# meiqua/pose_refine

Hardware: AMD Instinct MI355X
Metric: refined poses/sec (640x480, 20 ICP iters) (higher is better)
Workload: dtype f32; 1 GPU; obj_06.ply, 256-pose batch per GPU, 640x480 synthetic depth, projective association, 20 ICP iterations (21 passes), solve on device, 2 pose groups; poses_per_gpu=256, global_batch=256, parallelism=pose-shard x1, no data-path collective, no gather (1 rank)

## Files before the change

### pose_refine_amd/csrc/icp_accumulate.h

```cpp
#pragma once
#include "nn_query.h"

namespace prk {

struct Acc29 { float2v pk[16]; };
__device__ constexpr int kAccLo[16] = { 0, 6, 2, 7, 3, 8, 5, 11, 12, 24, 14, 15, 18, 17, 20, 27 };
__device__ constexpr int kAccHi[16] = { 1, -1, 21, 22, 4, 9, 10, 23, 13, 25, 26, 16, -1, 19, -1, 28 };
__device__ __forceinline__ void acc_clear(Acc29 &a) {
#pragma unroll
    for (int i = 0; i < 16; ++i) a.pk[i] = float2v{ 0.0f, 0.0f };
}
__device__ __forceinline__ void acc_export(const Acc29 &a, float (&out)[29]) {
#pragma unroll
    for (int i = 0; i < 16; ++i) { if (kAccLo[i] >= 0) out[kAccLo[i]] = a.pk[i].x; if (kAccHi[i] >= 0) out[kAccHi[i]] = a.pk[i].y; }
}
#define PR_SEL(v, i, j) __builtin_shufflevector(v, v, i, j)
__device__ __forceinline__ void accumulate(Acc29 &acc, float sx, float sy, float sz, const Corr &c)
{
    const float ex = c.dx - sx, ey = c.dy - sy, ez = c.dz - sz;
    const float r = ex * c.nx + ey * c.ny + ez * c.nz;
    const float2v C01{ c.nz * sy - c.ny * sz, c.nx * sz - c.nz * sx };
    const float2v C2R{ c.ny * sx - c.nx * sy, r };
    const float2v N01{ c.nx, c.ny };
    const float2v N2Z{ c.nz, c.dz };
// ... 49 lines not shown
    acc.pk[9]  += PR_SEL(WC2R, 1, 1) * N01;
    acc.pk[10] += WC2R * PR_SEL(N2Z, 0, 0);
    acc.pk[11] += PR_SEL(WN01, 0, 0) * N01;
    acc.pk[12] += PR_SEL(WN01, 1, 1) * PR_SEL(N01, 1, 0);
    acc.pk[13] += WN01 * PR_SEL(N2Z, 0, 0);
    acc.pk[14] += PR_SEL(WN2Z, 0, 0) * N2Z;
    acc.pk[15] += float2v{ e2, 1.0f };
    return w;
}
__device__ __forceinline__ void robust_store_corr(float *row, bool valid, const Corr &c, float w)
{
    const float4 a = valid ? make_float4(c.dx, c.dy, c.dz, 1.0f) : make_float4(0.0f, 0.0f, 0.0f, 0.0f);
    const float4 b = valid ? make_float4(c.nx, c.ny, c.nz, w) : make_float4(0.0f, 0.0f, 0.0f, 0.0f);
    reinterpret_cast<float4 *>(row)[0] = a;
    reinterpret_cast<float4 *>(row)[1] = b;
}
#undef PR_SEL

__device__ __forceinline__ void accumulate_score(Acc29 &acc, float sx, float sy, float sz, const Corr &c)
{
    const float ex = c.dx - sx, ey = c.dy - sy, ez = c.dz - sz;
    const float e2 = ex * ex + ey * ey + ez * ez;
    acc.pk[15] += float2v{ e2, 1.0f };
}


template <bool kScoreOnly, bool kRobust>
__device__ __forceinline__ void accumulate_point(Acc29 &acc, float sx, float sy, float sz, const Corr &c, const RobustW &rb)
{
    if constexpr (kScoreOnly) accumulate_score(acc, sx, sy, sz, c);
    else if constexpr (kRobust) (void)accumulate_weighted(acc, sx, sy, sz, c, rb);
    else accumulate(acc, sx, sy, sz, c);
}
template <class Scene, bool kNN, int kStack, bool kScoreOnly = false, bool kRobust = false>
__device__ __forceinline__ void vb_accumulate_at(uint32_t tib, float (&acc_out)[29], float *cl, uint32_t n, uint32_t first, uint32_t steps, bool xf,
                                                 const float (&M)[12], const Scene &scene, const int4 *lds_topo, int *stk_node, float *stk_lb,
                                                 uint32_t *nn_prev = nullptr, bool nn_seeded = false, const RobustW &rb = RobustW{})
{
    (void)nn_prev; (void)nn_seeded; (void)rb;
    struct { uint32_t steps; } b{ steps };
    Acc29 acc;
    acc_clear(acc);
    uint32_t lane_winner = kNoPrev;
    (void)lane_winner;
    (void)lds_topo; (void)stk_node; (void)stk_lb;
    auto point_of = [&](uint32_t j0, uint32_t i) { return j0 + i * kBlockThreads; };
    auto load_step = [&](uint32_t s, float (&p)[12], uint32_t &j0, uint32_t &cnt) {
        j0 = first + s * kPointsPerStep + tib;
        cnt = (j0 >= n) ? 0u : (((n - j0 + kBlockThreads - 1u) / kBlockThreads < kPointsPerLane) ? (n - j0 + kBlockThreads - 1u) / kBlockThreads : kPointsPerLane);
        const uint32_t last = n - 1u;
#pragma unroll
        for (uint32_t i = 0; i < 4; ++i) {
            const uint32_t j = point_of(j0, i);
            const pr_vec3 v = ld_off<pr_vec3>(cl, (j < last ? j : last) * 12u);
            p[3 * i] = v.x; p[3 * i + 1] = v.y; p[3 * i + 2] = v.z;
        }
    };
    auto process_step = [&](float (&p)[12], uint32_t j0, uint32_t cnt) {
        if (cnt == 0) return;
        if ((!kNN || kStack != -1) && xf) {
            const float2v Mx{ M[0], M[4] }, My{ M[1], M[5] }, Mz{ M[2], M[6] }, Mt{ M[3], M[7] };
#pragma unroll
            for (int i = 0; i < 4; ++i) {
                const float x = p[3 * i], y = p[3 * i + 1], z = p[3 * i + 2];
                float2v t = Mx * float2v{ x, x };
                t = t + My * float2v{ y, y };
                t = t + Mz * float2v{ z, z };
                t = t + Mt;
                p[3 * i]     = t.x;
                p[3 * i + 1] = t.y;
                p[3 * i + 2] = M[8] * x + M[9] * y + M[10] * z + M[11];
            }
#if !PR_PASS_LATE_STORE
#pragma unroll
            for (uint32_t i = 0; i < 4; ++i)
                if (i < cnt) st_off<pr_vec3>(cl, point_of(j0, i) * 12u, pr_vec3{ p[3 * i], p[3 * i + 1], p[3 * i + 2] });
#endif
        }
        auto store_back = [&]() {
#if PR_PASS_LATE_STORE
            if ((!kNN || kStack != -1) && xf) {
#pragma unroll
                for (uint32_t i = 0; i < 4; ++i)
                    if (i < cnt) st_off<pr_vec3>(cl, point_of(j0, i) * 12u, pr_vec3{ p[3 * i], p[3 * i + 1], p[3 * i + 2] });
            }
#endif
        };
        if constexpr (kNN) store_back();
        if constexpr (kNN && kStack == -1) {
            uint32_t w[4];
#pragma unroll
            for (uint32_t i = 0; i < 4; ++i) w[i] = (i < cnt) ? scene.winner[point_of(j0, i)] : kNoPrev;
            float4 d[4]; float nx[4], ny[4], nz[4];
#pragma unroll
            for (uint32_t i = 0; i < 4; ++i) {
                const uint32_t at = (w[i] != kNoPrev) ? w[i] : 0u;
                d[i] = scene.pts[at];
                const float *n = reinterpret_cast<const float *>(scene.normal + at);
                nx[i] = n[0]; ny[i] = n[1]; nz[i] = n[2];
            }
#pragma unroll
            for (uint32_t i = 0; i < 4; ++i) {
                if (w[i] != kNoPrev) {
                    Corr c; c.dx = d[i].x; c.dy = d[i].y; c.dz = d[i].z; c.nx = nx[i]; c.ny = ny[i]; c.nz = nz[i];
                    accumulate_point<kScoreOnly, kRobust>(acc, p[3 * i], p[3 * i + 1], p[3 * i + 2], c, rb);
                }
            }
        } else if constexpr (kNN) {
#pragma unroll
            for (uint32_t i = 0; i < 4; ++i) {
                if (i < cnt) {
                    Corr c;
                    bool ok;
                    if constexpr (kStack > 0) {
                        const uint32_t seed = (nn_prev && nn_seeded) ? nn_prev[point_of(j0, i)] : kNoPrev;
                        uint32_t winner;
                        ok = query_nn_stack<kStack>(scene, reinterpret_cast<const float4 *>(lds_topo), stk_node, stk_lb, p[3 * i], p[3 * i + 1], p[3 * i + 2], c,
// ... 28 lines not shown
    };

#if PR_PASS_PREFETCH
    {
        float p[12];
        uint32_t j0, cnt;
        load_step(0, p, j0, cnt);
        for (uint32_t s = 0; s < b.steps && cnt != 0; ++s) {
            float pn[12];
            uint32_t j0n = 0, cntn = 0;
            if (s + 1 < b.steps) load_step(s + 1, pn, j0n, cntn);
            process_step(p, j0, cnt);
#pragma unroll
            for (int i = 0; i < 12; ++i) p[i] = pn[i];
            j0 = j0n; cnt = cntn;
        }
    }
#else
    for (uint32_t s = 0; s < b.steps; ++s) {
        float p[12];
        uint32_t j0, cnt;
        load_step(s, p, j0, cnt);
        if (cnt == 0) break;
        process_step(p, j0, cnt);
    }
#endif
    acc_export(acc, acc_out);
}
template <class Scene, bool kNN, int kStack, bool kScoreOnly = false, bool kRobust = false>
__device__ __forceinline__ void vb_accumulate(float (&acc_out)[29], float *cl, uint32_t n, uint32_t first, uint32_t steps, bool xf,
                                              const float (&M)[12], const Scene &scene, const int4 *lds_topo, int *stk_node, float *stk_lb,
                                              uint32_t *nn_prev = nullptr, bool nn_seeded = false, const RobustW &rb = RobustW{})
{
    vb_accumulate_at<Scene, kNN, kStack, kScoreOnly, kRobust>(threadIdx.x, acc_out, cl, n, first, steps, xf, M, scene, lds_topo, stk_node, stk_lb, nn_prev, nn_seeded, rb);
}

template <bool kScoreOnly = false>
__device__ __forceinline__ void wave_reduce(float (&acc)[29], uint32_t lane, float *row)
{
    constexpr int kFirst = kScoreOnly ? 27 : 0;
#if PR_PASS_TAIL_PRIO
    __builtin_amdgcn_s_setprio(PR_PASS_TAIL_PRIO);
#endif
    if constexpr (!kScoreOnly) {
        const bool b1 = (lane & 1u) != 0, b2 = (lane & 2u) != 0;
        float p1[16], p2[8], p3[4], p4[2];
#pragma unroll
        for (int i = 0; i < 29; ++i) acc[i] += dpp_get<0x111, 0xf>(acc[i]);
#pragma unroll
        for (int k = 0; k < 15; ++k) {
            const float hi = acc[2 * k], lo = (2 * k + 1 < 29) ? dpp_get<0x101, 0xf>(acc[2 * k + 1 < 29 ? 2 * k + 1 : 28]) : 0.0f;
            p1[k] = b1 ? hi : lo;
        }
        p1[15] = 0.0f;
#pragma unroll
        for (int k = 0; k < 15; ++k) p1[k] += dpp_get<0x112, 0xf>(p1[k]);
#pragma unroll
        for (int m = 0; m < 8; ++m) {
            const float lo = dpp_get<0x102, 0xf>(p1[2 * m + 1]);
            p2[m] = b2 ? p1[2 * m] : lo;
        }
#pragma unroll
        for (int m = 0; m < 8; ++m) p2[m] += dpp_get<0x114, 0xf>(p2[m]);
#pragma unroll
        for (int q = 0; q < 4; ++q)
            p3[q] = __int_as_float(__builtin_amdgcn_update_dpp(__float_as_int(p2[2 * q]), __float_as_int(p2[2 * q + 1]), 0x104, 0xf, 0x5, false));
#pragma unroll
// ... 42 lines not shown
```

### pose_refine_amd/csrc/icp_pass.hip

```cpp
#include "pr_launch.h"
#include "icp_accumulate.h"
#include "icp_solve_device.h"

namespace prk {

template <class Scene, bool kNN, int kStack = 0, bool kRobust = false>
__global__ __launch_bounds__(256, PR_PASS_WAVES) void icp_pass_kernel(IcpBatch b, Scene scene)
{
    extern __shared__ __attribute__((aligned(16))) unsigned char lds_raw[];
    __shared__ float wsum[4][kAccStride];

    const uint32_t pose = blockIdx.y;
    const PoseMeta &pm = b.meta[pose];
    const int32_t st = pm.state;
    if (st == kSkip) return;
    const uint32_t n = pm.count;
    const uint32_t ppb = b.steps * kPointsPerStep;
    if ((uint64_t)blockIdx.x * ppb >= n) return;

    const int4 *lds_topo = nullptr;
    int *stk_node = nullptr; float *stk_lb = nullptr;
    if constexpr (kNN && kStack == 0) {
        int4 *dst = reinterpret_cast<int4 *>(lds_raw);
        for (uint32_t i = threadIdx.x; i < scene.lds_nodes; i += kBlockThreads) dst[i] = scene.topo[i];
// ... 25 lines not shown
        for (int i = 0; i < 29; ++i) acc[i] = 0.0f;
        float t;
        if (b.score_only) {
            vb_accumulate<Scene, kNN, kStack, true>(acc, cl, n, vb * ppb, b.steps, xf, M, scene, lds_topo, stk_node, stk_lb, nn_prev, xf);
            t = vb_reduce<true>(acc, wsum);
        } else {
            if constexpr (kRobust)
                vb_accumulate<Scene, kNN, kStack, false, true>(acc, cl, n, vb * ppb, b.steps, xf, M, scene, lds_topo, stk_node, stk_lb, nn_prev, xf, RobustW{ b.robust_kind, b.robust_c, b.robust_inv_c });
            else
                vb_accumulate<Scene, kNN, kStack>(acc, cl, n, vb * ppb, b.steps, xf, M, scene, lds_topo, stk_node, stk_lb, nn_prev, xf);
            t = vb_reduce(acc, wsum);
        }
        if (pass_deliver(b, pose, vb, used, n, t)) return;
    }
}

__device__ __forceinline__ float sum_partials(const float *partial, uint32_t pose, uint32_t nblk, uint32_t used, uint32_t comp)
{
    float total = 0.0f;
    const float *p = partial + (size_t)pose * nblk * kAccStride + comp;
    for (uint32_t g0 = 0; g0 < used; g0 += 16) {
        float v[16];
#pragma unroll
        for (uint32_t k = 0; k < 16; ++k) v[k] = (g0 + k < used) ? p[(size_t)(g0 + k) * kAccStride] : 0.0f;
#pragma unroll
        for (uint32_t k = 0; k < 16; ++k) if (g0 + k < used) total += v[k];
    }
    return total;
}

constexpr uint32_t kLoopLanes = 1024, kLoopWaves = kLoopLanes / 64, kLoopHeader = 64;
static_assert(sizeof(DevIcpState) == 20 * sizeof(uint32_t), "the LDS header holds DevIcpState as 20 words");
size_t icp_loop_cu_lds_bytes(uint32_t nblk) { return ((size_t)nblk * 4 * kAccStride + kLoopHeader) * sizeof(float); }

template <class Scene>
__global__ __launch_bounds__(kLoopLanes) PR_LOOP_CU_ATTR void icp_loop_cu_kernel(IcpBatch b, Scene scene)
{
    extern __shared__ __attribute__((aligned(16))) float loop_lds[];
    const uint32_t pose = blockIdx.x;
    const PoseMeta &pm = b.meta[pose];
    const int32_t st0 = pm.state;
    const uint32_t n = pm.count;
    if (st0 == kSkip || n == 0) return;
    const uint32_t ppb = b.steps * kPointsPerStep;
    const uint32_t items = ((n + ppb - 1) / ppb) * 4u;
    const uint32_t lane = threadIdx.x & 63u;
    const uint32_t wave = __builtin_amdgcn_readfirstlane(threadIdx.x >> 6);
    float *hdr = loop_lds + (size_t)b.nblk * 4 * kAccStride;
    uint32_t *hdw = reinterpret_cast<uint32_t *>(hdr);
    float *cl = reinterpret_cast<float *>(b.cloud + pm.start);
    bool xf = (st0 == kRunWithTransform) && !b.pre_transformed;
    float M[12];
#pragma unroll
    for (int i = 0; i < 12; ++i) M[i] = xf ? pm.xform[i] : 0.0f;
    if (wave == 0 && lane < 20) hdw[16 + lane] = reinterpret_cast<const uint32_t *>(b.st + pose)[lane];

    const uint32_t last_it = (uint32_t)b.crit.max_iteration;
    uint32_t it = 0;
    for (;; ++it) {
        const bool score_only = it == last_it;
        for (uint32_t item = wave; item < items; item += kLoopWaves) {
            const uint32_t vb = item >> 2, tib = ((item & 3u) << 6) | lane;
            float acc[29];
            float *row = loop_lds + (size_t)item * kAccStride;
            if (score_only) {
                vb_accumulate_at<Scene, false, 0, true>(tib, acc, cl, n, vb * ppb, b.steps, xf, M, scene, nullptr, nullptr, nullptr, nullptr, xf);
                wave_reduce<true>(acc, lane, row);
            } else {
                vb_accumulate_at<Scene, false, 0>(tib, acc, cl, n, vb * ppb, b.steps, xf, M, scene, nullptr, nullptr, nullptr, nullptr, xf);
                wave_reduce(acc, lane, row);
            }
        }
        __syncthreads();
        if (wave == 0) {
            float total = 0.0f;
            if (lane < 29) {
                const float *r = loop_lds + lane;
                for (uint32_t i = 0; i < items; i += 4u, r += 4 * kAccStride)
                    total += ((r[0] + r[kAccStride]) + r[2 * kAccStride]) + r[3 * kAccStride];
            }
            DevIcpState s;
#pragma unroll
            for (int i = 0; i < 16; ++i) s.T[i] = hdr[16 + i];
            s.fitness = hdr[32]; s.rmse = hdr[33]; s.done = (int32_t)hdw[34]; s.passes = (int32_t)hdw[35];
            float E[16];
            const bool finished = pose_iteration_wave(total, n, s, b.crit, it, E);
            if (lane == 0) {
#pragma unroll
                for (int i = 0; i < 16; ++i) hdr[16 + i] = s.T[i];
                hdr[32] = s.fitness; hdr[33] = s.rmse; hdw[35] = (uint32_t)s.passes;
                if (!finished) {
#pragma unroll
                    for (int i = 0; i < 12; ++i) hdr[i] = E[i];
                }
                hdw[12] = (finished || it >= last_it) ? 1u : 0u;
            }
        }
        __syncthreads();
        if (__builtin_amdgcn_readfirstlane(hdw[12]) != 0u) break;
#pragma unroll
        for (int i = 0; i < 12; ++i) M[i] = __int_as_float(__builtin_amdgcn_readfirstlane(__float_as_int(hdr[i])));
        xf = true;
    }
    if (threadIdx.x == 0) {
        DevIcpState s;
#pragma unroll
        for (int i = 0; i < 16; ++i) s.T[i] = hdr[16 + i];
        s.fitness = hdr[32]; s.rmse = hdr[33]; s.done = 1; s.passes = (int32_t)hdw[35];
        b.st[pose] = s;
        PoseMeta *wm = const_cast<PoseMeta *>(b.meta) + pose;
        if (it > 0) {
#pragma unroll
            for (int i = 0; i < 12; ++i) wm->xform[i] = hdr[i];
        }
        wm->state = kSkip;
    }
}
hipError_t launch_icp_loop_cu_proj_packed(const IcpBatch &b, const SceneProjPacked &sc, uint32_t n_poses, hipStream_t s)
{
    if (n_poses == 0 || b.nblk == 0) return hipSuccess;
    const size_t lds = icp_loop_cu_lds_bytes(b.nblk);
    if (lds > kLoopCuLdsBudget || b.robust_kind != PR_ROBUST_NONE) return hipErrorInvalidValue;
    hipLaunchKernelGGL(HIP_KERNEL_NAME(icp_loop_cu_kernel<SceneProjPacked>), dim3(n_poses), dim3(kLoopLanes), lds, s, b, sc);
    return hipGetLastError();
}

__global__ __launch_bounds__(64) void icp_finalize_kernel(const float *__restrict__ partial, const PoseMeta *__restrict__ meta,
                                                          uint32_t nblk, uint32_t ppb, float *__restrict__ sums)
{
    const uint32_t pose = blockIdx.x;
    if (meta[pose].state == kSkip) return;
    const uint32_t n = meta[pose].count;
    const uint32_t used = (n + ppb - 1) / ppb;
    if (threadIdx.x < kAccStride)
        sums[(size_t)pose * kAccStride + threadIdx.x] = (threadIdx.x < 29) ? sum_partials(partial, pose, nblk, used, threadIdx.x) : 0.0f;
}

__global__ __launch_bounds__(64) void icp_finalize_solve_kernel(const float *__restrict__ partial, PoseMeta *__restrict__ meta,
                                                                uint32_t nblk, uint32_t ppb, DevIcpState *__restrict__ st,
                                                                pr_criteria crit, uint32_t iter)
{
    const uint32_t pose = blockIdx.x;
    if (meta[pose].state == kSkip) return;
    const uint32_t n = meta[pose].count;
    const uint32_t used = (n + ppb - 1) / ppb;
    DevIcpState s = st[pose];
    float total = 0.0f;
    if (threadIdx.x < 29) total = sum_partials(partial, pose, nblk, used, threadIdx.x);
    float E[16];
    const bool finished = pose_iteration_wave(total, n, s, crit, iter, E);
    if (threadIdx.x != 0) return;
    if (finished) { s.done = 1; meta[pose].state = kSkip; }
    else {
#pragma unroll
        for (int i = 0; i < 12; ++i) meta[pose].xform[i] = E[i];
        meta[pose].state = kRunWithTransform;
// ... 129 lines not shown
```

### pose_refine_amd/csrc/pr_context.cpp

```cpp
#include "pr_runtime.h"

namespace prh {
thread_local std::string g_err;
void set_error(const char *fmt, ...)
{
    char buf[512];
    va_list ap; va_start(ap, fmt); vsnprintf(buf, sizeof buf, fmt, ap); va_end(ap);
    g_err = buf;
}
}

namespace prr {

static std::mutex &g_reg_mu_trace() { static std::mutex m; return m; }

namespace {
struct TraceRec { uint64_t ns; const char *tag; uint32_t tid; };
constexpr size_t kTraceCap = 1u << 18;
TraceRec *g_trace = nullptr;
std::atomic<uint64_t> g_trace_n{ 0 };
std::atomic<int> g_trace_state{ 0 };
std::string g_trace_path;
void trace_dump()
{
    FILE *f = std::fopen(g_trace_path.c_str(), "w");
    if (!f) return;
    const uint64_t n = std::min<uint64_t>(g_trace_n.load(), kTraceCap);
    for (uint64_t i = 0; i < n; ++i) std::fprintf(f, "%llu %u %s\n", (unsigned long long)g_trace[i].ns, g_trace[i].tid, g_trace[i].tag);
    std::fclose(f);
}
}
void trace_mark(const char *tag)
{
    int st = g_trace_state.load(std::memory_order_acquire);
    if (st == 1) return;
    if (st == 0) {
        std::lock_guard<std::mutex> lk(g_reg_mu_trace());
        st = g_trace_state.load();
        if (st == 0) {
            const char *p = std::getenv("PR_TRACE");
            if (p && *p) { g_trace_path = p; g_trace = new TraceRec[kTraceCap]; std::atexit(trace_dump); st = 2; } else st = 1;
            g_trace_state.store(st, std::memory_order_release);
        }
        if (st == 1) return;
    }
    timespec ts; clock_gettime(CLOCK_MONOTONIC, &ts);
    static thread_local uint32_t tid = (uint32_t)std::hash<std::thread::id>()(std::this_thread::get_id());
    const uint64_t i = g_trace_n.fetch_add(1);
    if (i < kTraceCap) g_trace[i] = TraceRec{ (uint64_t)ts.tv_sec * 1000000000ull + (uint64_t)ts.tv_nsec, tag, tid };
}

WriteLog g_writes;
std::atomic<uint64_t> g_flag_overtook{ 0 };
std::atomic<uint64_t> g_tight_batches{ 0 };
std::atomic<uint64_t> g_band_batches{ 0 };
std::atomic<uint64_t> g_resident_batches{ 0 };
Options opt;
std::mutex g_reg_mu;
std::vector<Ctx *> g_shared;
int g_default_device = -1;
thread_local Ctx *g = nullptr;
thread_local PrivateCtx tl_private;
std::mutex g_private_mu;
std::vector<Ctx *> g_private;

void ctx_teardown(Ctx *c)
{
    if (!c->ready) return;
    (void)hipSetDevice(c->device);
    hipStreamSynchronize(c->stream);
    for (Slot &sl : c->slots) slot_release(sl);
    for (DevBuf *b : { &c->aabb, &c->aabb_keys, &c->bbox, &c->poses, &c->depth, &c->row_count, &c->row_off, &c->counts, &c->cloud, &c->meta, &c->partial,
                       &c->sums, &c->packed.rec, &c->nn_prev, &c->dstate, &c->dresults, &c->arrive, &c->conv16, &c->conv8, &c->kd_scratch, &c->kd_tmp, &c->nn_full, &c->gather_tmp, &c->nn_counters, &c->scores, &c->multi, &c->ov_bits, &c->ov_box, &c->ov_mat, &c->cov_state, &c->cov_claimed, &c->mesh_sorted, &c->mesh_verts, &c->contours, &c->normals, &c->cmp_keys, &c->cmp_box, &c->cmp_rec, &c->edge_bits, &c->edge_rows, &c->lvl_rows, &c->lvl_counts, &c->lvl_carry, &c->pd_mats, &c->pd_part, &c->pd_rec, &c->ppf_tmp, &c->ppf_out, &c->plane_tmp, &c->seg_tmp, &c->dfilt_tmp, &c->vsd_rec, &c->solid_far, &c->solid_rec, &c->info_meta, &c->info_part }) b->release();
    for (NNDerived &d : c->nn_sets) d.release();
    for (PinBuf *b : { &c->h_sums, &c->h_meta, &c->h_counts, &c->h_results, &c->h_dstate, &c->h_poses, &c->h_flags, &c->h_scores, &c->h_multi, &c->h_ov, &c->h_cov, &c->h_contours, &c->h_normals, &c->h_lvl_carry, &c->h_cmp, &c->h_pd_mats, &c->h_pd_rec, &c->h_ppf, &c->h_plane, &c->h_seg, &c->h_dfilt, &c->h_vsd, &c->h_solid, &c->h_info_meta, &c->h_info_out }) b->release();
    c->packed = PackedCache();
    for (auto &gr : c->graphs) destroy_graph(gr);
    c->graphs.clear();
    c->spans.destroy();
    for (auto &e : c->gather_ev) { hipEventDestroy(e.first); hipEventDestroy(e.second); }
    c->gather_ev.clear(); c->gather_ev_used = 0;
    hipStreamDestroy(c->stream);
    if (c->ev_fork) hipEventDestroy(c->ev_fork);
    c->ev_fork = nullptr;
    for (int i = 0; i < 3; ++i) {
        if (c->side[i]) hipStreamDestroy(c->side[i]);
        if (c->ev_join[i]) hipEventDestroy(c->ev_join[i]);
        c->side[i] = nullptr; c->ev_join[i] = nullptr;
    }
// ... 166 lines not shown
    note_write(dev_dst, count * sizeof(int32_t));
    HIP_TRY(prk::launch_fill_i32(dev_dst, count, value, g->stream));
    HIP_TRY(hipStreamSynchronize(g->stream));
    return PR_OK;
}

int pr_set_option(const char *name, int value)
{
    std::lock_guard<std::mutex> lk(g_reg_mu);
    if (!name) { set_error("pr_set_option: null name"); return PR_ERR_INVALID; }
    const std::string n(name);
    if (n == "solve") { if (value != PR_SOLVE_HOST && value != PR_SOLVE_DEVICE) { set_error("solve must be 0 or 1"); return PR_ERR_INVALID; } opt.solve_mode = value; }
    else if (n == "host_worker") opt.host_worker = value ? 1 : 0;
    else if (n == "start_overlap") opt.start_overlap = value;
    else if (n == "points_per_block") { if (value < 1024 || value % 1024) { set_error("points_per_block must be a multiple of 1024"); return PR_ERR_INVALID; } opt.steps = value / 1024; }
    else if (n == "profile") { if (value < 0 || value > 3) { set_error("profile must be 0, 1 (every launch, synchronous calls), 2 (every launch of one call in sample_period) or 3 (every launch, asynchronous batches stay asynchronous)"); return PR_ERR_INVALID; } opt.profile = value; }
    else if (n == "sample_period") opt.sample_period = std::max(1, value);
    else if (n == "scene_cache") opt.scene_cache = value ? 1 : 0;
    else if (n == "nn_lds_nodes") opt.nn_lds_nodes = std::max(0, value);
    else if (n == "nn_lds_records") opt.nn_lds_records = std::max(0, value);
    else if (n == "nn_compact") opt.nn_compact = value ? 1 : 0;
    else if (n == "nn_wide") opt.nn_wide = value ? 1 : 0;
    else if (n == "blocking_wait") opt.blocking_wait = value ? 1 : 0;
    else if (n == "nn_seed") opt.nn_seed = value ? 1 : 0;
    else if (n == "nn_stack") opt.nn_stack = value ? 1 : 0;
    else if (n == "nn_split") opt.nn_split = value ? 1 : 0;
    else if (n == "nn_run") opt.nn_run = std::min(256, std::max(1, value));
    else if (n == "nn_grid") opt.nn_grid = value ? 1 : 0;
    else if (n == "nn_count") opt.nn_count = value ? 1 : 0;
    else if (n == "host_poll") opt.host_poll = value ? 1 : 0;
    else if (n == "graph") opt.use_graph = value ? 1 : 0;
    else if (n == "fused_solve") opt.fused_solve = value ? 1 : 0;
    else if (n == "resident_loop") opt.resident_loop = value ? 1 : 0;
    else if (n == "sub_batch") opt.sub_batch = std::min(32768, std::max(32, value));
    else if (n == "overlap_pass") opt.overlap_pass = std::max(-1, value);
    else if (n == "pose_groups") opt.pose_groups = std::min(4, std::max(0, value));
    else if (n == "eager_streams") opt.eager_streams = value ? 1 : 0;
    else if (n == "mesh_order") opt.mesh_order = value ? 1 : 0;
    else if (n == "tight_box") opt.tight_box = value ? 1 : 0;
    else if (n == "box_bands") opt.box_bands = value ? 1 : 0;
    else if (n == "ppf_walk") opt.ppf_walk = value ? 1 : 0;
    else if (n == "raster_mode") { if (value < 0 || value > 1) { set_error("raster_mode must be 0 or 1"); return PR_ERR_INVALID; } opt.raster_mode = value; }
    else { set_error("unknown option %s", name); return PR_ERR_INVALID; }
    return PR_OK;
}

int pr_get_option(const char *name, int *value)
{
    std::lock_guard<std::mutex> lk(g_reg_mu);
    if (!name || !value) { set_error("pr_get_option: null argument"); return PR_ERR_INVALID; }
    const std::string n(name);
    if (n == "solve") *value = opt.solve_mode;
    else if (n == "host_worker") *value = opt.host_worker;
    else if (n == "start_overlap") *value = opt.start_overlap;
    else if (n == "points_per_block") *value = opt.steps * 1024;
    else if (n == "profile") *value = opt.profile;
    else if (n == "sample_period") *value = opt.sample_period;
    else if (n == "scene_cache") *value = opt.scene_cache;
    else if (n == "nn_lds_nodes") *value = opt.nn_lds_nodes;
    else if (n == "nn_lds_records") *value = opt.nn_lds_records;
    else if (n == "nn_compact") *value = opt.nn_compact;
    else if (n == "nn_wide") *value = opt.nn_wide;
    else if (n == "blocking_wait") *value = opt.blocking_wait;
    else if (n == "nn_seed") *value = opt.nn_seed;
    else if (n == "nn_stack") *value = opt.nn_stack;
    else if (n == "nn_split") *value = opt.nn_split;
    else if (n == "nn_run") *value = opt.nn_run;
    else if (n == "nn_grid") *value = opt.nn_grid;
    else if (n == "nn_count") *value = opt.nn_count;
    else if (n == "host_poll") *value = opt.host_poll;
    else if (n == "stat_flag_overtook") *value = (int)std::min<uint64_t>(g_flag_overtook.load(), 0x7fffffffull);
    else if (n == "stat_tight_batches") *value = (int)std::min<uint64_t>(g_tight_batches.load(), 0x7fffffffull);
    else if (n == "box_pack") *value = (int)prk::kBoxPack;
    else if (n == "pose_dist_chunk") *value = (int)prk::kPoseDistChunk;
    else if (n == "raster_mode") *value = opt.raster_mode;
    else if (n == "mesh_order") *value = opt.mesh_order;
    else if (n == "tight_box") *value = opt.tight_box;
    else if (n == "box_bands") *value = opt.box_bands;
    else if (n == "ppf_walk") *value = opt.ppf_walk;
    else if (n == "stat_band_batches") *value = (int)std::min<uint64_t>(g_band_batches.load(), 0x7fffffffull);
    else if (n == "eager_streams") *value = opt.eager_streams;
    else if (n == "graph") *value = opt.use_graph;
    else if (n == "fused_solve") *value = opt.fused_solve;
    else if (n == "resident_loop") *value = opt.resident_loop;
    else if (n == "stat_resident_batches") *value = (int)std::min<uint64_t>(g_resident_batches.load(), 0x7fffffffull);
    else if (n == "sub_batch") *value = opt.sub_batch;
    else if (n == "overlap_pass") *value = opt.overlap_pass;
    else if (n == "pose_groups") *value = opt.pose_groups;
    else { set_error("unknown option %s", name); return PR_ERR_INVALID; }
    return PR_OK;
}

int pr_profile_reset(void)
{
    PR_TRY(bind_default());
    std::lock_guard<std::mutex> lk(g->mu);
    g->icp_ms = g->render_ms = g->cloud_ms = 0; g->icp_launches = g->icp_points = g->icp_bytes = 0; g->sample_clock = 0;
    g->gather_ms = 0; g->gather_n = 0; g->gather_ev_used = 0;
    g->icp_launch_us.clear();
    for (double &v : g->nn_part_ms) v = 0;
    g->nn_part_n = 0;
    return PR_OK;
}

int pr_stats(uint64_t *batches_repeated, uint64_t *timings_dropped)
{
    PR_TRY(bind_default());
    std::lock_guard<std::mutex> lk(g->mu);
    if (batches_repeated) *batches_repeated = g->stat_repeated;
    if (timings_dropped) *timings_dropped = g->stat_timing_dropped;
    return PR_OK;
}

int pr_profile_launches(float *launch_us, uint32_t capacity, uint32_t *n)
{
    PR_TRY(bind_default());
    std::lock_guard<std::mutex> lk(g->mu);
// ... 30 lines not shown
```

### pose_refine_amd/csrc/pr_internal.h

```cpp
#pragma once

#include <hip/hip_runtime_api.h>
#include <hip/hip_vector_types.h>
#include <stddef.h>
#include <stdint.h>
#include <vector>

#include "pose_refine.h"
#include "pr_tuning.h"

namespace prk {

constexpr uint32_t kBlockThreads   = 256;
constexpr uint32_t kPointsPerLane  = 4;
constexpr uint32_t kPointsPerStep  = kBlockThreads * kPointsPerLane;
constexpr uint32_t kAccStride      = 32;
constexpr uint32_t kCloudAlign     = 32;
constexpr uint32_t kBoxPack        = 32;
constexpr uint32_t kQCountStride   = 4;
constexpr uint32_t kNNWordsPerPoint = 6;

enum : int32_t { kSkip = 0, kRun = 1, kRunWithTransform = 2 };

struct alignas(64) PoseMeta {
// ... 1 lines not shown
    uint32_t count;
    int32_t  state;
    uint32_t pad;
    float    xform[12];
};
static_assert(sizeof(PoseMeta) == 64, "PoseMeta must stay one 64-byte record");

struct DevIcpState;
struct IcpBatch {
    pr_vec3        *cloud;
    const PoseMeta *meta;
    float          *partial;
    uint32_t        nblk;
    uint32_t        grid_x;
    uint32_t        steps;
    uint32_t        score_only;
    uint32_t        fused;
    float          *sums_out;
    uint32_t       *grp_count;
    uint32_t        grp_expected;
    uint32_t       *grp_flag;
    uint32_t        iter;
    DevIcpState    *st;
    uint32_t       *arrive;
    uint32_t       *nn_prev;
    float          *nn_slack;
    uint2          *nn_queue;
    uint32_t       *nn_qcount;
    uint2          *nn_queue2;
    uint32_t        pre_transformed;
    pr_criteria     crit;
    uint32_t        robust_kind;
    float           robust_c, robust_inv_c;
};
struct RobustArgs { uint32_t kind; float c, inv_c; float *corr; };

struct SceneProjAoS {
    uint32_t width, height;
    float max_dist_diff, fx, fy, cx, cy;
    float tlx, tly;
    const pr_vec3 *pcd, *normal;
};
struct SceneProjPacked {
    uint32_t width, height;
    float max_dist_diff, fx, fy, cx, cy;
    float tlx, tly;
    const float4 *rec;
    const float *colf, *rowf;
};
struct SceneNNDev {
    float max_dist_diff;
    const int4   *topo;
    const float4 *bmin, *bmax;
    const float4 *pts;
    const pr_vec3 *pcd, *normal;
    uint32_t n_nodes;
    uint32_t lds_nodes;
    const float4 *rec;
    uint32_t stack_depth;
    const uint4 *rec32;
    float qmin[3], qscale[3];
    const uint2 *desc;
    const float4 *grid;
    uint32_t gw, gh;
    float gfx, gfy, gcx, gcy;
    const float4 *pyr4, *pyr16, *pyr64;
// ... 130 lines not shown
struct PoseDistCamera { float fx, cx, fy, cy; };
hipError_t launch_pose_dist(const pr_vec3 *points, uint32_t n_points, const double *as_rows, const float *b_rows, uint32_t n_b, uint32_t n_k,
                            uint32_t pair0, uint32_t n_pairs, bool all_pairs, const PoseDistCamera *cam, uint32_t n_rows, uint32_t chunks_per_row,
                            void *partials, hipStream_t s);
hipError_t launch_pose_dist_combine(const void *partials, uint32_t n_rows, uint32_t n_pairs, uint32_t n_k, uint32_t n_points, bool with_proj,
                                    pr_pose_dist *records, hipStream_t s);
struct VsdPairing { uint32_t est_mul, gt_mul, gt_add; };
struct VsdParams { float delta; uint32_t n_taus; float tau[PR_VSD_MAX_TAUS]; uint32_t has_k; float fx, cx, fy, cy; };
hipError_t launch_vsd_boxes(const int32_t *depth, const int4 *bbox, const uint32_t *box_off, uint32_t n_pairs, const VsdPairing &pairing, uint32_t width,
                            uint32_t height, const void *scene, bool scene_i32, const VsdParams &pm, uint32_t *records, hipStream_t s);
hipError_t launch_pack_export(const DevIcpState *st, pr_result *out, const uint32_t *counts, uint32_t *host_counts, pr_result *host_results,
                              uint32_t n, hipStream_t s);
hipError_t launch_stage_words(const void *src_host_mapped, void *dst, size_t bytes, hipStream_t s);
hipError_t launch_stage_words64(const void *src_host_mapped, void *dst, size_t bytes, hipStream_t s);
hipError_t launch_copy_words32(const void *src, void *dst, uint32_t n_words, hipStream_t s);
hipError_t launch_d2c_pack_starts(const uint32_t *counts, uint32_t n, PoseMeta *meta, hipStream_t s);
hipError_t launch_emit_box(const int32_t *depth, uint32_t n_poses, uint32_t width, uint32_t height, const int4 *bbox, float fx, float fy,
                           float cx, float cy, const uint32_t *row_count, const uint32_t *row_off, pr_vec3 *cloud, const PoseMeta *meta,
                           hipStream_t s, const uint32_t *box_off = nullptr, bool bands = false);

struct PyramidStrides { uint32_t n; uint32_t s[PR_PYRAMID_MAX_LEVELS]; };
struct alignas(64) PyramidCarry { float T[12]; uint32_t start; uint32_t pad[3]; };
static_assert(sizeof(PyramidCarry) == 64, "PyramidCarry must stay one 64-byte record");
hipError_t launch_pyramid_counts(const int32_t *depth, const int4 *bbox, const uint32_t *box_off, uint32_t n_poses, uint32_t width, uint32_t height,
                                 const PyramidStrides &lv, uint32_t *row_count, uint32_t *row_off, uint32_t *counts, hipStream_t s);
hipError_t launch_pyramid_emit(const int32_t *depth, uint32_t n_poses, uint32_t width, uint32_t height, const int4 *bbox, const uint32_t *box_off,
                               float fx, float fy, float cx, float cy, uint32_t stride, const uint32_t *row_count, const uint32_t *row_off,
                               const PyramidCarry *carry, bool apply, pr_vec3 *cloud, hipStream_t s);

hipError_t launch_icp_pass_proj_aos(const IcpBatch &b, const SceneProjAoS &sc, uint32_t n_poses, hipStream_t s);
hipError_t launch_icp_pass_proj_packed(const IcpBatch &b, const SceneProjPacked &sc, uint32_t n_poses, hipStream_t s);
constexpr size_t kLoopCuLdsBudget = 64u << 10;
size_t icp_loop_cu_lds_bytes(uint32_t nblk);
hipError_t launch_icp_loop_cu_proj_packed(const IcpBatch &b, const SceneProjPacked &sc, uint32_t n_poses, hipStream_t s);
hipError_t launch_icp_pass_nn(const IcpBatch &b, const SceneNNDev &sc, uint32_t n_poses, hipStream_t s);
hipError_t launch_nn_search(const IcpBatch &b, const SceneNNDev &sc, uint32_t n_poses, uint32_t max_points, uint32_t run, hipStream_t s, hipEvent_t *marks = nullptr);
hipError_t launch_icp_pass_nn_winners(const IcpBatch &b, const SceneNNWinners &sc, uint32_t n_poses, hipStream_t s);
hipError_t launch_icp_pass_grid(const IcpBatch &b, const SceneGridDev &sc, uint32_t n_poses, hipStream_t s);
hipError_t launch_grid_build(const SceneNNDev &tree, float reach, const SceneGridDev &grid, uint32_t *cell_point, hipStream_t s);
hipError_t launch_grid_records(const pr_vec3 *pcd, const pr_vec3 *normal, uint32_t n, float4 *rec, hipStream_t s);
hipError_t launch_contrib29_grid(pr_vec3 *cloud, uint32_t n, const float *update12, const SceneGridDev &sc, float *out, hipStream_t s);
hipError_t launch_contrib29_proj_aos(pr_vec3 *cloud, uint32_t n, const float *update12, const SceneProjAoS &sc, float *out, hipStream_t s);
hipError_t launch_contrib29_proj_packed(pr_vec3 *cloud, uint32_t n, const float *update12, const SceneProjPacked &sc, float *out, hipStream_t s);
hipError_t launch_contrib29_nn(pr_vec3 *cloud, uint32_t n, const float *update12, const SceneNNDev &sc, float *out, hipStream_t s);
hipError_t launch_robust_terms_proj_aos(pr_vec3 *cloud, uint32_t n, const float *update12, const SceneProjAoS &sc, const RobustArgs &ra, float *out, hipStream_t s);
hipError_t launch_robust_terms_proj_packed(pr_vec3 *cloud, uint32_t n, const float *update12, const SceneProjPacked &sc, const RobustArgs &ra, float *out, hipStream_t s);
hipError_t launch_robust_terms_nn(pr_vec3 *cloud, uint32_t n, const float *update12, const SceneNNDev &sc, const RobustArgs &ra, float *out, hipStream_t s);
hipError_t launch_robust_terms_grid(pr_vec3 *cloud, uint32_t n, const float *update12, const SceneGridDev &sc, const RobustArgs &ra, float *out, hipStream_t s);
hipError_t launch_pose_iteration_debug(const float *sums, const uint32_t *n_points, uint32_t n, pr_criteria crit, uint32_t iter, pr_result *state,
                                       float *update, uint32_t *finished, hipStream_t s);
size_t nn_grid_cells(uint32_t gw, uint32_t gh);
hipError_t launch_build_nn_grid(const pr_vec3 *pcd, uint32_t n_points, uint32_t gw, uint32_t gh, float fx, float fy, float cx, float cy,
                                int32_t *cell_idx, float4 *grid, uint32_t *usable, hipStream_t s);
hipError_t launch_icp_finalize(const float *partial, const PoseMeta *meta, uint32_t nblk,
                               uint32_t steps, float *sums, uint32_t n_poses, hipStream_t s);
hipError_t launch_icp_finalize_solve(const float *partial, PoseMeta *meta, uint32_t nblk,
                                     uint32_t steps, DevIcpState *st, pr_criteria crit, uint32_t iter,
                                     uint32_t n_poses, hipStream_t s);
hipError_t launch_pack_results(const DevIcpState *st, pr_result *out, uint32_t n_poses, hipStream_t s);

struct KdLevelNode { int left, right, child, axis; float cut; int pad0, pad1, pad2; };
struct KdCtrl { uint32_t lo, hi, next, done, levels, error, pad0, pad1; };
struct KdWork {
    void *base = nullptr;
    KdCtrl *ctrl[2] = { nullptr, nullptr };
    int *idx[2] = { nullptr, nullptr }, *owner[2] = { nullptr, nullptr };
    KdLevelNode *lv[2] = { nullptr, nullptr };
// ... 70 lines not shown
```

### pose_refine_amd/csrc/pr_refine.cpp

```cpp
#include "pr_runtime.h"
#include "pose_box.h"

namespace prr {

int stage_poses(const pr_mat4 *poses_host, size_t n)
{
    PR_TRY(g->poses.ensure(sizeof(pr_mat4) * n));
    PR_TRY(g->h_poses.ensure(sizeof(pr_mat4) * n));
    std::memcpy(g->h_poses.p, poses_host, sizeof(pr_mat4) * n);
    HIP_TRY(prk::launch_stage_words(g->h_poses.dev, g->poses.p, sizeof(pr_mat4) * n, g->stream));
    return PR_OK;
}

uint32_t depth_chunk(size_t img, uint32_t P)
{
    return (uint32_t)std::max<size_t>(1, std::min<size_t>(P, ((size_t)4 << 30) / (img * sizeof(int32_t))));
}

std::pair<size_t, size_t> image_extent(pr_roi roi, size_t W, size_t H)
{
    if (roi.width > 0 && roi.height > 0) return { (size_t)roi.width, (size_t)roi.height };
    return { W, H };
}

// ... 899 lines not shown
    prk::PoseMeta *meta = sl.meta.as<prk::PoseMeta>() + q0;
    prk::DevIcpState *dstate = sl.dstate.as<prk::DevIcpState>() + q0;
    uint32_t *arrive = sl.arrive.as<uint32_t>() + q0;
    const pr_roi none{ 0, 0, 0, 0 };
    size_t te = timed ? sl.spans.begin(st) : kNoEvent;
    if (q0 == 0) HIP_TRY(hipStreamWaitEvent(st, sl.scene_ready, 0));
    if (tight) HIP_TRY(prk::launch_box_pack_offsets(d_box + q0, nq, d_off + q0, H, bands, st));
    prk::RasterMesh mesh{};
    mesh.tris = raster_tris; mesh.n_tris = (uint32_t)job.mesh.n_tris;
    prk::RasterTarget target{};
    target.depth = sl.depth.as<int32_t>(); target.box_off = d_off + q0; target.roi = none; target.bands = bands; target.width = W; target.height = H; target.proj = &job.proj;
    const prk::BoxRows rows{ sl.row_count.as<uint32_t>(), sl.row_off.as<uint32_t>(), sl.counts.as<uint32_t>() + q0, meta, dstate, arrive };
    HIP_TRY(prk::launch_render_boxes(mesh, d_poses + q0, nq, d_box + q0, target, rows, st, false, q0 == 0 ? &chk : nullptr));
    if (timed) { sl.spans.end(te, kSpanRender, q0, nq, false, st); te = sl.spans.begin(st); }
    HIP_TRY(prk::launch_emit_box(sl.depth.as<int32_t>(), nq, W, H, d_box + q0, K[0], K[4], K[2], K[5], sl.row_count.as<uint32_t>(),
                                 sl.row_off.as<uint32_t>(), sl.cloud.as<pr_vec3>(), meta, st, d_off + q0, bands));
    if (timed) sl.spans.end(te, kSpanCloud, q0, nq, false, st);
    if (timed && q0 == 0)
        for (Slot &o : g->slots) if (&o != &sl && o.pending && !o.delivered && o.done) HIP_TRY(hipStreamWaitEvent(st, o.done, 0));

    const uint32_t n_groups = pose_group_count(job.scene_kind, nq, timed);
    if (nn_prev) HIP_TRY(prk::launch_fill_i32(reinterpret_cast<int32_t *>(nn_prev + nl.qcount), (size_t)prk::kQCountStride * nq, 0, st));
    prk::IcpBatch b{};
    b.cloud = sl.cloud.as<pr_vec3>(); b.partial = sl.partial.as<float>(); b.nblk = pl.nblk; b.grid_x = pl.grid_x; b.steps = pl.steps;
    if (nn_prev) nn_carve(b, nn_prev, nl);
    const uint32_t last_pass = (uint32_t)job.crit.max_iteration;
    if (opt.resident_loop && opt.fused_solve && !timed && job.scene_kind == PR_SCENE_PROJ && sc.kind == PR_SCENE_PROJ && sc.packed
        && prk::icp_loop_cu_lds_bytes(pl.nblk) <= prk::kLoopCuLdsBudget) {
        b.meta = meta; b.st = dstate; b.crit = job.crit; b.fused = 1;
        const bool release = q0 + pl.sub >= P;
#if PR_RESIDENT_RELEASE_AHEAD
        if (release) { HIP_TRY(hipEventRecord(sl.progress, st)); sl.progress_valid = true; }
#endif
        HIP_TRY(prk::launch_icp_loop_cu_proj_packed(b, sc.pk, nq, st));
#if !PR_RESIDENT_RELEASE_AHEAD
        if (release) { HIP_TRY(hipEventRecord(sl.progress, st)); sl.progress_valid = true; }
#endif
        g_resident_batches.fetch_add(1);
        return PR_OK;
    }
    auto pass = [&](const prk::IcpBatch &bb, uint32_t p0, uint32_t np, hipStream_t gs) -> int {
        if (!timed) { HIP_TRY(launch_pass(bb, sc, np, gs)); return PR_OK; }
        const size_t e0 = sl.spans.begin(st);
        size_t mi[3] = { 0, 0, 0 }; hipEvent_t me[3] = { nullptr, nullptr, nullptr };
        const bool marks = sc.kind == PR_SCENE_NN && sc.nn_split && bb.nn_prev && np <= 32768u && sl.spans.reserve_marks(mi, me);
        HIP_TRY(launch_pass(bb, sc, np, gs, marks ? me : nullptr));
        sl.spans.end(e0, kSpanIcp, q0 + p0, np, bb.iter == 0 || bb.iter == last_pass, st, marks ? mi : nullptr);
        return PR_OK;
    };
    const uint32_t release_pass = release_pass_for(job.mesh.n_tris, nq, g->cloud_hint, job.crit, job.scene_kind, timed, pipeline_start, opt.start_overlap, opt.overlap_pass);
    auto after = [&](uint32_t it, bool &) -> int {
        if (q0 + pl.sub >= P && it == release_pass) { HIP_TRY(hipEventRecord(sl.progress, st)); sl.progress_valid = true; }
        return PR_OK;
    };
    const Lanes lanes{ sl.stream, sl.side, sl.fork, sl.join };
    return device_solve_loop(lanes, n_groups, b, nq, job.crit, opt.fused_solve != 0, meta, dstate, arrive, pass, after);
}
int refine_submit_async(Slot &sl, const RefineJob &job, uint32_t P, pr_result *results_host)
{
    AsyncBatch a{ sl, job, P };
    hipStream_t scene_stream = nullptr;
    PR_TRY(async_scene(sl, job, P, a.sc, scene_stream));
    PR_TRY(ensure_model_box(job.mesh.tris, job.mesh.n_tris));
    const SlotIn in(P);
    const SlotOut out(P);
    PR_TRY(sl.h_out.ensure(out.bytes));
    unsigned char *h_out_dev = sl.h_out.dev_as<unsigned char>();
// ... 609 lines not shown
```

### pose_refine_amd/csrc/pr_runtime.h

```cpp
#pragma once
#include <hip/hip_runtime_api.h>
#include <rccl/rccl.h>
#include <dlfcn.h>

#include <algorithm>
#include <atomic>
#include <cfloat>
#include <cmath>
#include <cstdarg>
#include <cstdio>
#include <cstdlib>
#include <cstring>
#include <condition_variable>
#include <memory>
#include <mutex>
#include <thread>
#include <string>
#include <vector>

#include "pr_internal.h"
#include "pr_tuning.h"
#include "pose_box.h"
#include "contour_fit.h"

// ... 56 lines not shown
struct WriteLog {
    std::mutex mu;
    struct W { uintptr_t lo, hi; };
    static constexpr uint64_t kRing = 128;
    W ring[kRing];
    uint64_t gen = 0;
    void note(const void *p, size_t bytes)
    {
        if (!p) return;
        uintptr_t lo = reinterpret_cast<uintptr_t>(p), hi = lo + bytes;
        if (bytes == 0) {
            void *base = nullptr; size_t size = 0;
            if (hipMemGetAddressRange(reinterpret_cast<hipDeviceptr_t *>(&base), &size, const_cast<void *>(p)) == hipSuccess && base) { lo = reinterpret_cast<uintptr_t>(base); hi = lo + size; }
            else { (void)hipGetLastError(); lo = 0; hi = ~(uintptr_t)0; }
        }
        std::lock_guard<std::mutex> lk(mu);
        ++gen;
        ring[gen % kRing] = W{ lo, hi };
    }
    uint64_t now() { std::lock_guard<std::mutex> lk(mu); return gen; }
    bool written_since(uint64_t since, const void *p, size_t bytes)
    {
        const uintptr_t lo = reinterpret_cast<uintptr_t>(p), hi = lo + bytes;
        std::lock_guard<std::mutex> lk(mu);
        if (gen - since >= kRing) return true;
        for (uint64_t k = since + 1; k <= gen; ++k) { const W &w = ring[k % kRing]; if (w.lo < hi && lo < w.hi) return true; }
        return false;
    }
};
extern WriteLog g_writes;
extern std::atomic<uint64_t> g_tight_batches;
extern std::atomic<uint64_t> g_band_batches;
extern std::atomic<uint64_t> g_resident_batches;
extern std::atomic<uint64_t> g_flag_overtook;

constexpr int kSlots = PR_SLOTS;
struct Options {
    int pose_groups = 0;
    int solve_mode = PR_SOLVE_HOST;
    int host_worker = 1;
    int steps = 3;
    int profile = 0;
    int sample_period = 32;
    int nn_lds_nodes = 1024;
    int nn_lds_records = 0;
    int nn_seed = 1;
    int nn_compact = 1;
    int blocking_wait = 0;
    int nn_wide = 1;
    int nn_stack = 1;
    int nn_split = 1;
    int nn_run = 8;
    int nn_grid = 1;
    int host_poll = 1;
    int nn_count = 0;
    int start_overlap = -1;
    int overlap_pass = -1;
    int sub_batch = 512;
    int fused_solve = 1;
    int resident_loop = 1;
    int use_graph = 1;
    int eager_streams = 1;
    int raster_mode = 0;
    int mesh_order = 1;
    int tight_box = 1;
    int box_bands = 1;
    int ppf_walk = 1;
    int scene_cache = 1;
};
extern Options opt;
inline uint32_t pose_groups_for(int scene_kind) { (void)scene_kind; return opt.pose_groups > 0 ? (uint32_t)opt.pose_groups : 2u; }

struct ProjTail { uint32_t exact; prk::FpWords fp; uint32_t pad[3]; };
static_assert(sizeof(ProjTail) == 32, "ProjTail: the 32 bytes behind the tables");
struct PackedLayout { size_t colf, rowf, tail, bytes; };
inline PackedLayout packed_layout(size_t w, size_t h)
{
    PackedLayout l{};
    l.colf = w * h * sizeof(float4); l.rowf = l.colf + w * sizeof(float);
    l.tail = l.colf + (((w + h) * sizeof(float) + 15) & ~(size_t)15); l.bytes = l.tail + sizeof(ProjTail);
    return l;
}
struct PackedCache {
    DevBuf rec;
    template <class T> T *at(size_t offset) const { return reinterpret_cast<T *>(static_cast<unsigned char *>(rec.p) + offset); }
    const void *pcd = nullptr, *normal = nullptr;
    uint64_t w = 0, h = 0; float k[4] = { 0, 0, 0, 0 }; uint32_t tl[2] = { 0, 0 };
    uint64_t gen = 0;
    bool valid = false, exact = false;
};
inline bool frame_size_ok(size_t W, size_t H)
{
    if (W > 8192 || H > 8192 || W * H > ((size_t)1 << 24)) { set_error("frames larger than 8192 on a side or 2^24 pixels are not supported (got %zux%zu)", W, H); return false; }
// ... 807 lines not shown
```

Baseline: 331,100 poses/s.

## Keep transformed cloud blocks resident in LDS across resident-loop ICP iterations

In the per-CU resident ICP loop kernel, as many leading virtual blocks of the transformed point cloud as fit in extended LDS (up to 160 KiB, opt-in) are copied into LDS on the first iteration. Later iterations read and write those points from LDS instead of global memory. This targets the global read and write-back traffic for the cloud on every pass. In exchange each CU needs more LDS, which may reduce occupancy, and the launch depends on the large-LDS opt-in succeeding.

```diff
diff --git a/pose_refine_amd/csrc/icp_accumulate.h b/pose_refine_amd/csrc/icp_accumulate.h
--- a/pose_refine_amd/csrc/icp_accumulate.h
+++ b/pose_refine_amd/csrc/icp_accumulate.h
@@ -105,8 +105,8 @@
     else if constexpr (kRobust) (void)accumulate_weighted(acc, sx, sy, sz, c, rb);
     else accumulate(acc, sx, sy, sz, c);
 }
-template <class Scene, bool kNN, int kStack, bool kScoreOnly = false, bool kRobust = false>
-__device__ __forceinline__ void vb_accumulate_at(uint32_t tib, float (&acc_out)[29], float *cl, uint32_t n, uint32_t first, uint32_t steps, bool xf,
+template <class Scene, bool kNN, int kStack, bool kScoreOnly = false, bool kRobust = false, bool kStoreAlways = false>
+__device__ __forceinline__ void vb_accumulate_at(uint32_t tib, float (&acc_out)[29], const float *src, float *dst, uint32_t n, uint32_t first, uint32_t steps, bool xf,
                                                  const float (&M)[12], const Scene &scene, const int4 *lds_topo, int *stk_node, float *stk_lb,
                                                  uint32_t *nn_prev = nullptr, bool nn_seeded = false, const RobustW &rb = RobustW{})
 {
@@ -125,13 +125,14 @@
 #pragma unroll
         for (uint32_t i = 0; i < 4; ++i) {
             const uint32_t j = point_of(j0, i);
-            const pr_vec3 v = ld_off<pr_vec3>(cl, (j < last ? j : last) * 12u);
+            const pr_vec3 v = ld_off<pr_vec3>(src, (j < last ? j : last) * 12u);
             p[3 * i] = v.x; p[3 * i + 1] = v.y; p[3 * i + 2] = v.z;
         }
     };
     auto process_step = [&](float (&p)[12], uint32_t j0, uint32_t cnt) {
         if (cnt == 0) return;
-        if ((!kNN || kStack != -1) && xf) {
+        const bool moved = (!kNN || kStack != -1) && xf, put = kStoreAlways || moved;
+        if (moved) {
             const float2v Mx{ M[0], M[4] }, My{ M[1], M[5] }, Mz{ M[2], M[6] }, Mt{ M[3], M[7] };
 #pragma unroll
             for (int i = 0; i < 4; ++i) {
@@ -144,18 +145,20 @@
                 p[3 * i + 1] = t.y;
                 p[3 * i + 2] = M[8] * x + M[9] * y + M[10] * z + M[11];
             }
+        }
 #if !PR_PASS_LATE_STORE
+        if (put) {
 #pragma unroll
             for (uint32_t i = 0; i < 4; ++i)
-                if (i < cnt) st_off<pr_vec3>(cl, point_of(j0, i) * 12u, pr_vec3{ p[3 * i], p[3 * i + 1], p[3 * i + 2] });
+                if (i < cnt) st_off<pr_vec3>(dst, point_of(j0, i) * 12u, pr_vec3{ p[3 * i], p[3 * i + 1], p[3 * i + 2] });
+        }
 #endif
-        }
         auto store_back = [&]() {
 #if PR_PASS_LATE_STORE
-            if ((!kNN || kStack != -1) && xf) {
+            if (put) {
 #pragma unroll
                 for (uint32_t i = 0; i < 4; ++i)
-                    if (i < cnt) st_off<pr_vec3>(cl, point_of(j0, i) * 12u, pr_vec3{ p[3 * i], p[3 * i + 1], p[3 * i + 2] });
+                    if (i < cnt) st_off<pr_vec3>(dst, point_of(j0, i) * 12u, pr_vec3{ p[3 * i], p[3 * i + 1], p[3 * i + 2] });
             }
 #endif
         };
@@ -250,7 +253,7 @@
                                               const float (&M)[12], const Scene &scene, const int4 *lds_topo, int *stk_node, float *stk_lb,
                                               uint32_t *nn_prev = nullptr, bool nn_seeded = false, const RobustW &rb = RobustW{})
 {
-    vb_accumulate_at<Scene, kNN, kStack, kScoreOnly, kRobust>(threadIdx.x, acc_out, cl, n, first, steps, xf, M, scene, lds_topo, stk_node, stk_lb, nn_prev, nn_seeded, rb);
+    vb_accumulate_at<Scene, kNN, kStack, kScoreOnly, kRobust>(threadIdx.x, acc_out, cl, cl, n, first, steps, xf, M, scene, lds_topo, stk_node, stk_lb, nn_prev, nn_seeded, rb);
 }
 
 template <bool kScoreOnly = false>
diff --git a/pose_refine_amd/csrc/icp_pass.hip b/pose_refine_amd/csrc/icp_pass.hip
--- a/pose_refine_amd/csrc/icp_pass.hip
+++ b/pose_refine_amd/csrc/icp_pass.hip
@@ -81,6 +81,15 @@
 constexpr uint32_t kLoopLanes = 1024, kLoopWaves = kLoopLanes / 64, kLoopHeader = 64;
 static_assert(sizeof(DevIcpState) == 20 * sizeof(uint32_t), "the LDS header holds DevIcpState as 20 words");
 size_t icp_loop_cu_lds_bytes(uint32_t nblk) { return ((size_t)nblk * 4 * kAccStride + kLoopHeader) * sizeof(float); }
+uint32_t icp_loop_cu_lds_blocks(uint32_t nblk, uint32_t steps, int cap)
+{
+    const size_t fixed = icp_loop_cu_lds_bytes(nblk), block = (size_t)steps * kPointsPerStep * sizeof(pr_vec3);
+    if (fixed > kLoopCuLdsBudget || block == 0) return 0;
+    const size_t fit = (kLoopCuLdsTotal - fixed) / block;
+    uint32_t r = (uint32_t)(fit < nblk ? fit : nblk);
+    if (cap >= 0 && (uint32_t)cap < r) r = (uint32_t)cap;
+    return r;
+}
 
 template <class Scene>
 __global__ __launch_bounds__(kLoopLanes) PR_LOOP_CU_ATTR void icp_loop_cu_kernel(IcpBatch b, Scene scene)
@@ -98,6 +107,8 @@
     float *hdr = loop_lds + (size_t)b.nblk * 4 * kAccStride;
     uint32_t *hdw = reinterpret_cast<uint32_t *>(hdr);
     float *cl = reinterpret_cast<float *>(b.cloud + pm.start);
+    float *lcl = hdr + kLoopHeader;
+    const uint32_t lds_items = b.lds_blocks * 4u;
     bool xf = (st0 == kRunWithTransform) && !b.pre_transformed;
     float M[12];
 #pragma unroll
@@ -112,11 +123,16 @@
             const uint32_t vb = item >> 2, tib = ((item & 3u) << 6) | lane;
             float acc[29];
             float *row = loop_lds + (size_t)item * kAccStride;
+            const bool in_lds = item < lds_items;
             if (score_only) {
-                vb_accumulate_at<Scene, false, 0, true>(tib, acc, cl, n, vb * ppb, b.steps, xf, M, scene, nullptr, nullptr, nullptr, nullptr, xf);
+                if (!in_lds) vb_accumulate_at<Scene, false, 0, true>(tib, acc, cl, cl, n, vb * ppb, b.steps, xf, M, scene, nullptr, nullptr, nullptr, nullptr, xf);
+                else if (it == 0) vb_accumulate_at<Scene, false, 0, true, false, true>(tib, acc, cl, lcl, n, vb * ppb, b.steps, xf, M, scene, nullptr, nullptr, nullptr, nullptr, xf);
+                else vb_accumulate_at<Scene, false, 0, true>(tib, acc, lcl, lcl, n, vb * ppb, b.steps, xf, M, scene, nullptr, nullptr, nullptr, nullptr, xf);
                 wave_reduce<true>(acc, lane, row);
             } else {
-                vb_accumulate_at<Scene, false, 0>(tib, acc, cl, n, vb * ppb, b.steps, xf, M, scene, nullptr, nullptr, nullptr, nullptr, xf);
+                if (!in_lds) vb_accumulate_at<Scene, false, 0>(tib, acc, cl, cl, n, vb * ppb, b.steps, xf, M, scene, nullptr, nullptr, nullptr, nullptr, xf);
+                else if (it == 0) vb_accumulate_at<Scene, false, 0, false, false, true>(tib, acc, cl, lcl, n, vb * ppb, b.steps, xf, M, scene, nullptr, nullptr, nullptr, nullptr, xf);
+                else vb_accumulate_at<Scene, false, 0>(tib, acc, lcl, lcl, n, vb * ppb, b.steps, xf, M, scene, nullptr, nullptr, nullptr, nullptr, xf);
                 wave_reduce(acc, lane, row);
             }
         }
@@ -165,12 +181,21 @@
         wm->state = kSkip;
     }
 }
-hipError_t launch_icp_loop_cu_proj_packed(const IcpBatch &b, const SceneProjPacked &sc, uint32_t n_poses, hipStream_t s)
-{
+hipError_t launch_icp_loop_cu_proj_packed(const IcpBatch &b, const SceneProjPacked &sc, uint32_t n_poses, hipStream_t s, uint32_t *lds_blocks_used)
+{
+    if (lds_blocks_used) *lds_blocks_used = 0;
     if (n_poses == 0 || b.nblk == 0) return hipSuccess;
-    const size_t lds = icp_loop_cu_lds_bytes(b.nblk);
+    size_t lds = icp_loop_cu_lds_bytes(b.nblk);
     if (lds > kLoopCuLdsBudget || b.robust_kind != PR_ROBUST_NONE) return hipErrorInvalidValue;
-    hipLaunchKernelGGL(HIP_KERNEL_NAME(icp_loop_cu_kernel<SceneProjPacked>), dim3(n_poses), dim3(kLoopLanes), lds, s, b, sc);
+    IcpBatch bb = b;
+    const uint32_t most = icp_loop_cu_lds_blocks(b.nblk, b.steps, -1);
+    if (bb.lds_blocks > most) bb.lds_blocks = most;
+    const size_t image = (size_t)bb.lds_blocks * b.steps * kPointsPerStep * sizeof(pr_vec3);
+    const auto fn = icp_loop_cu_kernel<SceneProjPacked>;
+    if (lds + image > kLoopCuLdsBudget && !lds_opt_in(reinterpret_cast<const void *>(fn), 0, (uint32_t)kLoopCuLdsTotal)) bb.lds_blocks = 0;
+    if (bb.lds_blocks) lds += image;
+    if (lds_blocks_used) *lds_blocks_used = bb.lds_blocks;
+    hipLaunchKernelGGL(HIP_KERNEL_NAME(icp_loop_cu_kernel<SceneProjPacked>), dim3(n_poses), dim3(kLoopLanes), lds, s, bb, sc);
     return hipGetLastError();
 }
 
diff --git a/pose_refine_amd/csrc/pr_context.cpp b/pose_refine_amd/csrc/pr_context.cpp
--- a/pose_refine_amd/csrc/pr_context.cpp
+++ b/pose_refine_amd/csrc/pr_context.cpp
@@ -55,6 +55,7 @@
 std::atomic<uint64_t> g_tight_batches{ 0 };
 std::atomic<uint64_t> g_band_batches{ 0 };
 std::atomic<uint64_t> g_resident_batches{ 0 };
+std::atomic<uint32_t> g_loop_lds_blocks{ 0 };
 Options opt;
 std::mutex g_reg_mu;
 std::vector<Ctx *> g_shared;
@@ -287,6 +288,7 @@
     else if (n == "graph") opt.use_graph = value ? 1 : 0;
     else if (n == "fused_solve") opt.fused_solve = value ? 1 : 0;
     else if (n == "resident_loop") opt.resident_loop = value ? 1 : 0;
+    else if (n == "loop_lds_blocks") opt.loop_lds_blocks = std::max(-1, value);
     else if (n == "sub_batch") opt.sub_batch = std::min(32768, std::max(32, value));
     else if (n == "overlap_pass") opt.overlap_pass = std::max(-1, value);
     else if (n == "pose_groups") opt.pose_groups = std::min(4, std::max(0, value));
@@ -338,6 +340,8 @@
     else if (n == "graph") *value = opt.use_graph;
     else if (n == "fused_solve") *value = opt.fused_solve;
     else if (n == "resident_loop") *value = opt.resident_loop;
+    else if (n == "loop_lds_blocks") *value = opt.loop_lds_blocks;
+    else if (n == "stat_loop_lds_blocks") *value = (int)g_loop_lds_blocks.load();
     else if (n == "stat_resident_batches") *value = (int)std::min<uint64_t>(g_resident_batches.load(), 0x7fffffffull);
     else if (n == "sub_batch") *value = opt.sub_batch;
     else if (n == "overlap_pass") *value = opt.overlap_pass;
diff --git a/pose_refine_amd/csrc/pr_internal.h b/pose_refine_amd/csrc/pr_internal.h
--- a/pose_refine_amd/csrc/pr_internal.h
+++ b/pose_refine_amd/csrc/pr_internal.h
@@ -57,6 +57,7 @@
     pr_criteria     crit;
     uint32_t        robust_kind;
     float           robust_c, robust_inv_c;
+    uint32_t        lds_blocks;
 };
 struct RobustArgs { uint32_t kind; float c, inv_c; float *corr; };
 
@@ -253,7 +254,9 @@
 hipError_t launch_icp_pass_proj_packed(const IcpBatch &b, const SceneProjPacked &sc, uint32_t n_poses, hipStream_t s);
 constexpr size_t kLoopCuLdsBudget = 64u << 10;
 size_t icp_loop_cu_lds_bytes(uint32_t nblk);
-hipError_t launch_icp_loop_cu_proj_packed(const IcpBatch &b, const SceneProjPacked &sc, uint32_t n_poses, hipStream_t s);
+constexpr size_t kLoopCuLdsTotal = 160u << 10;
+uint32_t icp_loop_cu_lds_blocks(uint32_t nblk, uint32_t steps, int cap);
+hipError_t launch_icp_loop_cu_proj_packed(const IcpBatch &b, const SceneProjPacked &sc, uint32_t n_poses, hipStream_t s, uint32_t *lds_blocks_used = nullptr);
 hipError_t launch_icp_pass_nn(const IcpBatch &b, const SceneNNDev &sc, uint32_t n_poses, hipStream_t s);
 hipError_t launch_nn_search(const IcpBatch &b, const SceneNNDev &sc, uint32_t n_poses, uint32_t max_points, uint32_t run, hipStream_t s, hipEvent_t *marks = nullptr);
 hipError_t launch_icp_pass_nn_winners(const IcpBatch &b, const SceneNNWinners &sc, uint32_t n_poses, hipStream_t s);
diff --git a/pose_refine_amd/csrc/pr_refine.cpp b/pose_refine_amd/csrc/pr_refine.cpp
--- a/pose_refine_amd/csrc/pr_refine.cpp
+++ b/pose_refine_amd/csrc/pr_refine.cpp
@@ -955,7 +955,10 @@
 #if PR_RESIDENT_RELEASE_AHEAD
         if (release) { HIP_TRY(hipEventRecord(sl.progress, st)); sl.progress_valid = true; }
 #endif
-        HIP_TRY(prk::launch_icp_loop_cu_proj_packed(b, sc.pk, nq, st));
+        b.lds_blocks = prk::icp_loop_cu_lds_blocks(pl.nblk, pl.steps, opt.loop_lds_blocks);
+        uint32_t lds_blocks_used = 0;
+        HIP_TRY(prk::launch_icp_loop_cu_proj_packed(b, sc.pk, nq, st, &lds_blocks_used));
+        g_loop_lds_blocks.store(lds_blocks_used);
 #if !PR_RESIDENT_RELEASE_AHEAD
         if (release) { HIP_TRY(hipEventRecord(sl.progress, st)); sl.progress_valid = true; }
 #endif
diff --git a/pose_refine_amd/csrc/pr_runtime.h b/pose_refine_amd/csrc/pr_runtime.h
--- a/pose_refine_amd/csrc/pr_runtime.h
+++ b/pose_refine_amd/csrc/pr_runtime.h
@@ -112,6 +112,7 @@
 extern std::atomic<uint64_t> g_tight_batches;
 extern std::atomic<uint64_t> g_band_batches;
 extern std::atomic<uint64_t> g_resident_batches;
+extern std::atomic<uint32_t> g_loop_lds_blocks;
 extern std::atomic<uint64_t> g_flag_overtook;
 
 constexpr int kSlots = PR_SLOTS;
@@ -139,6 +140,7 @@
     int sub_batch = 512;
     int fused_solve = 1;
     int resident_loop = 1;
+    int loop_lds_blocks = -1;
     int use_graph = 1;
     int eager_streams = 1;
     int raster_mode = 0;
```

New measurement: 346,100 poses/s, median of 6. 1.05x the previous value.
